# Koukyosyumei/MyZKP

Hardware: AMD Instinct MI355X
Metric: G1 MSM pairs/sec + NTT elems/sec at 2^20 and 2^24; bit-exact vs CPU (higher is better)
Workload: dtype u32x9 (29-bit limbs, 254-bit Montgomery); 1 GPU; KZG commit = BN254 G1 Pippenger MSM of 2^20 (scalar, point) pairs per GPU against a device-resident SRS (commit_kzg, kzg.rs:57-59); 17-bit signed windows (library default at this size), 15 window tables built once at upload; N GPUs = one MSM of N*2^20 pairs (BASELINE configs[2]/[3]); pairs_per_gpu=1048576, seed=332211571536, window_bits=17

## Files before the change

myzkp_amd/csrc/mzk_common.h:

```cpp
#pragma once
#include <hip/hip_runtime.h>
#include <stdint.h>
#include <stddef.h>
#include <stdio.h>
#include <string.h>
#include <functional>
#include <string>
#include <vector>
#include "../../include/mzk.h"
#include "mzk_field.h"
#include "mzk_msm_plan.h"
#include "mzk_ws.h"

namespace mzk {

#ifdef MZK_TUNING
#include <stdlib.h>
static inline int tune_int(const char* name, int dflt) { const char* v = getenv(name); return v ? atoi(v) : dflt; } static inline const char* tune_str(const char* name) { return getenv(name); }
#else
static inline constexpr int tune_int(const char*, int dflt) { return dflt; }
static inline constexpr const char* tune_str(const char*) { return nullptr; }
#endif

void set_error(const char* fmt, ...);
void clear_error();
size_t table_budget_bytes();
int hip_fail(hipError_t e, const char* what, const char* file, int line);
#define MZK_HIP(x)                                                        \
  do {                                                                    \
    hipError_t _e = (x);                                                  \
    if (_e != hipSuccess) return mzk::hip_fail(_e, #x, __FILE__, __LINE__); \
  } while (0)
#define MZK_TRY(x)        \
  do {                    \
    int _rc = (x);        \
    if (_rc != MZK_OK) return _rc; \
  } while (0)

enum AttrFlag { ATTR_FINE_SCATTER4 = 0, ATTR_FINE_SCATTER8, ATTR_DIGITS_LDS, ATTR_SMALL_MSM, ATTR_NTT_LARGE_FR, ATTR_NTT_LARGE_M128, ATTR_NTT_LARGE_M128_2WG, ATTR_MANY_SORT1, ATTR_TAIL_ROW, ATTR_COARSE_STAGED4, ATTR_COARSE_STAGED8, ATTR_COUNT };
struct Context {
  bool ready = false;
  int index = 0;
  int device = -1;
  int num_cu = 256;
  hipStream_t stream = nullptr;
  WsTable ws;
  hipEvent_t ws_event = nullptr;
  hipEvent_t fork_event = nullptr, join_event = nullptr;
  hipStream_t ws_last = nullptr;
  bool ws_used = false;
  bool attr_done[ATTR_COUNT] = {};
  hipStream_t xstream[MZK_MAX_CTX] = {};
  hipEvent_t xdone[MZK_MAX_CTX] = {};
  hipEvent_t xready = nullptr;
  void* bounce = nullptr;
};
constexpr size_t SMALL_D2H_MAX = 4096;
int d2h_sync(void* host, const void* dev, size_t bytes, hipStream_t s);
int ctx_peer_enabled(int a, int b);
struct EntryGuard {
  bool ok;
  bool nested;
  EntryGuard();
  ~EntryGuard();
};
#define MZK_ENTER()                        \
  mzk::EntryGuard _mzk_entry;              \
  if (!_mzk_entry.ok) return MZK_E_BUSY;   \
  MZK_TRY(mzk::ensure_init())
Context& ctx();
int ctx_count();
int ctx_select(int index);
int ensure_init();
struct CtxScope {
  int prev_ctx, prev_dev; bool ok;
  explicit CtxScope(int index);
  ~CtxScope();
};

struct WsGuard {
  hipStream_t s;
  explicit WsGuard(hipStream_t s_);
  ~WsGuard();
};

void prof_begin(hipStream_t s, int phase);
void prof_end(hipStream_t s, int phase);
struct ProfScope {
  hipStream_t s; int ph;
  ProfScope(hipStream_t s_, int ph_) : s(s_), ph(ph_) { prof_begin(s, ph); }
  ~ProfScope() { prof_end(s, ph); }
};
// ... 175 lines not shown
```

myzkp_amd/csrc/mzk_msm.hip:

```cpp
#include <stdlib.h>
#include <type_traits>
#include "mzk_common.h"
#include "mzk_elem.h"
#include "mzk_ec.h"
#include "mzk_coop.h"
#include "mzk_row.h"
#include "mzk_glv.h"
#include "mzk_affine_wave.h"

namespace mzk {

static const MsmKnobs& msm_knobs() {
  static const MsmKnobs k = [] {
    const MsmKnobs d;
    return MsmKnobs{tune_int("MZK_GLV_C", d.glv_c), tune_int("MZK_SMALL_SCAN", d.small_scan), tune_int("MZK_SCAN_MAX_LOG", d.scan_max_log),
                    tune_int("MZK_ACC_SEG", d.acc_seg), tune_int("MZK_COARSE_LOG_20", d.coarse_log_20),
                    tune_int("MZK_COARSE_LOG_17", d.coarse_log_17), tune_int("MZK_PER_FINE", d.per_fine), tune_int("MZK_SORT_SCAN_FREE", d.sort_scan_free),
                    tune_int("MZK_COMBINE_WIDE_MIN_LOG", d.combine_wide_min_log), tune_int("MZK_COMBINE_FORM", d.combine_form),
                    tune_int("MZK_COMBINE_LANE_TPB", d.combine_lane_tpb)};
  }();
  return k;
}

int msm_generic_window_bits(size_t n) { return choose_shape_glv(n ? n : 1, msm_knobs().glv_c).c; }

__device__ __forceinline__ Xyzz xyzz_gload(const u32* __restrict__ g, size_t idx) {
  u32 w[32];
#pragma unroll
  for (int q = 0; q < 4; q++) load_words8(g + idx * 32 + 8 * q, w + 8 * q);
  return xyzz_load(w);
}
__device__ __forceinline__ void xyzz_gstore(u32* __restrict__ g, size_t idx, const Xyzz& p) {
  u32 w[32];
  xyzz_store(p, w);
#pragma unroll
  for (int q = 0; q < 4; q++) store_words8(g + idx * 32 + 8 * q, w + 8 * q);
}

static_assert(SLOT_WORDS == 4 * FqParams::L, "a slot is the four raw coordinates");
__device__ __forceinline__ void xyzz_gstore_raw(u32* __restrict__ g, size_t idx, const Xyzz& p) {
  u32 w[SLOT_WORDS];
  const bool inf = xyzz_is_inf(p);
#pragma unroll
  for (int i = 0; i < FqParams::L; i++) {
    w[i] = inf ? 0u : p.X.l[i]; w[9 + i] = inf ? 0u : p.Y.l[i]; w[18 + i] = inf ? 0u : p.ZZ.l[i]; w[27 + i] = inf ? 0u : p.ZZZ.l[i];
  }
  uint4* p4 = reinterpret_cast<uint4*>(g + idx * SLOT_WORDS);
#pragma unroll
  for (int q = 0; q < SLOT_WORDS / 4; q++) p4[q] = make_uint4(w[4 * q], w[4 * q + 1], w[4 * q + 2], w[4 * q + 3]);
}
__device__ __forceinline__ Xyzz xyzz_gload_raw(const u32* __restrict__ g, size_t idx) {
  u32 w[SLOT_WORDS];
  const uint4* p4 = reinterpret_cast<const uint4*>(g + idx * SLOT_WORDS);
#pragma unroll
  for (int q = 0; q < SLOT_WORDS / 4; q++) { const uint4 v = p4[q]; w[4 * q] = v.x; w[4 * q + 1] = v.y; w[4 * q + 2] = v.z; w[4 * q + 3] = v.w; }
  Xyzz p;
#pragma unroll
  for (int i = 0; i < FqParams::L; i++) { p.X.l[i] = w[i]; p.Y.l[i] = w[9 + i]; p.ZZ.l[i] = w[18 + i]; p.ZZZ.l[i] = w[27 + i]; }
  return p;
}
__device__ __forceinline__ Xyzz xyzz_gload_raw_quad(const u32* __restrict__ g, size_t idx, int lane) {
  Fq mine;
  const u32* src = g + idx * SLOT_WORDS + 9 * lane;
#pragma unroll
  for (int i = 0; i < FqParams::L; i++) mine.l[i] = src[i];
  Xyzz p;
  p.X = quad_bcast<0>(mine);
  p.Y = quad_bcast<1>(mine);
  p.ZZ = quad_bcast<2>(mine);
  p.ZZZ = quad_bcast<3>(mine);
  return p;
}
// ... 370 lines not shown
  for (int k = 0; k < COARSE_PER_WG / SORT2_THREADS; k++) {
    const size_t i = lo + tid + (size_t)k * SORT2_THREADS;
    if (i < hi) load_scalar_canonical(scalars, i, w[k]);
  }
#pragma unroll 1
  for (int k = 0; k < COARSE_PER_WG / SORT2_THREADS; k++) {
    const size_t i = lo + tid + (size_t)k * SORT2_THREADS;
    if (tid < COARSE_BINS) hist[tid] = 0;
    __syncthreads();
    if (i < hi) walk_digits_merged<C>(w[k], table_stride, i, [&](int, u32 key, u32) { counter_inc_agg(hist, key >> key_shift); });
    __syncthreads();
    if (tid < 64) {
      u32 c[PER_LANE], sum = 0;
#pragma unroll
      for (int q = 0; q < PER_LANE; q++) { c[q] = hist[PER_LANE * tid + q]; sum += c[q]; }
      u32 incl = sum;
#pragma unroll
      for (int d = 1; d < 64; d <<= 1) {
        const u32 up = (u32)__shfl_up((int)incl, d, 64);
        if (tid >= d) incl += up;
      }
      u32 run = incl - sum;
#pragma unroll
      for (int q = 0; q < PER_LANE; q++) { loff[PER_LANE * tid + q] = run; run += c[q]; }
      if (tid == 63) loff[COARSE_BINS] = incl;
    }
    __syncthreads();
    if (tid < COARSE_BINS) {
      const u32 cnt = hist[tid];
      if (bin_tot) {
        gpos[tid] = cursor[tid] + (cnt ? atomicAdd(&bin_cur[tid], cnt) : 0u);
      } else {
        gpos[tid] = cursor[tid];
        cursor[tid] += cnt;
      }
      hist[tid] = loff[tid];
    }
    __syncthreads();
    if (i < hi) walk_digits_merged<C>(w[k], table_stride, i, [&](int, u32 key, u32 payload) {
      const u32 bin = key >> key_shift;
      const u32 pos = counter_inc_agg(hist, bin);
      stage[pos] = REC::make(payload, key & fine_mask, fb);
      stage_bin[pos] = (BinTag)bin;
    });
    __syncthreads();
    const u32 total = loff[COARSE_BINS];
    for (u32 p = tid; p < total; p += SORT2_THREADS) {
      const u32 b = stage_bin[p];
      tmp[gpos[b] + (p - loff[b])] = stage[p];
    }
    __syncthreads();
  }
}
struct FineSlice { int bin, s, Sb; u32 lo, hi, start; bool active; };
__device__ __forceinline__ FineSlice fine_plan(const u32* __restrict__ binbase, int nwg, int bins, int S, u32 cap, u32* sc, u32* res) {
  const int tid = threadIdx.x;
  u32 start = 0, len = 0, Sb = 0;
  if (tid < bins) {
    start = binbase[(size_t)tid * nwg];
    len = binbase[(size_t)(tid + 1) * nwg] - start;
    Sb = (len + cap - 1) / cap;
    if (Sb < (u32)S) Sb = (u32)S;
  }
  if (tid == 0) res[0] = 0xffffffffu;
  const int lane = tid & 63, wave = tid >> 6;
  u32 v = Sb;
#pragma unroll
  for (int off = 1; off < 64; off <<= 1) { const u32 t = __shfl_up(v, off, 64); if (lane >= off) v += t; }
  if (lane == 63) sc[wave] = v;
  __syncthreads();
  if (wave == 0) {
    u32 t = (lane < SORT2_THREADS / 64) ? sc[lane] : 0u;
#pragma unroll
    for (int off = 1; off < SORT2_THREADS / 64; off <<= 1) { const u32 u = __shfl_up(t, off, 64); if (lane >= off) t += u; }
    if (lane < SORT2_THREADS / 64) sc[lane] = t;
  }
  __syncthreads();
  const u32 w = blockIdx.x, incl = v + (wave ? sc[wave - 1] : 0u), excl = incl - Sb;
  if (tid < bins && excl <= w && w < incl) { res[0] = (u32)tid; res[1] = w - excl; res[2] = Sb; res[3] = start; res[4] = len; res[5] = excl; }
  __syncthreads();
  FineSlice r;
  r.active = res[0] != 0xffffffffu;
  r.bin = (int)res[0]; r.s = (int)res[1]; r.Sb = (int)res[2];
  const u64 L = res[4];
  r.start = res[3];
  r.lo = res[3] + (u32)(L * (u64)r.s / (u64)r.Sb);
  r.hi = res[3] + (u32)(L * (u64)(r.s + 1) / (u64)r.Sb);
  return r;
}
constexpr int FINE_UNROLL = 8;
template <class REC>
__global__ __launch_bounds__(SORT2_THREADS) void k_fine_count(const typename REC::T* __restrict__ tmp, const u32* __restrict__ binbase, int nwg, int F,
                                                               int S, int fb, u32* __restrict__ finehist, int bins, u32 cap, u32* __restrict__ bucket_tot) {
  __shared__ u32 hist[FINE_MAX];
  __shared__ u32 sc[SORT2_THREADS];
  const FineSlice p = fine_plan(binbase, nwg, bins, S, cap, sc, hist);
  __syncthreads();
  if (!p.active) {
    for (int f = threadIdx.x; f < F; f += SORT2_THREADS) finehist[(size_t)blockIdx.x * F + f] = 0;
    return;
  }
  for (int f = threadIdx.x; f < F; f += SORT2_THREADS) hist[f] = 0;
  __syncthreads();
  const u32 lo = p.lo, hi = p.hi;
  for (u32 base = lo + threadIdx.x; base < hi; base += FINE_UNROLL * SORT2_THREADS) {
    u32 f[FINE_UNROLL];
#pragma unroll
    for (int k = 0; k < FINE_UNROLL; k++) {
      const u32 e = base + k * SORT2_THREADS;
      f[k] = (e < hi) ? REC::fine(tmp[e], (u32)F - 1u, fb) : 0xffffffffu;
    }
#pragma unroll
    for (int k = 0; k < FINE_UNROLL; k++) if (f[k] != 0xffffffffu) counter_inc_agg(hist, f[k]);
  }
  __syncthreads();
  const size_t hbase = (size_t)F * (blockIdx.x - (u32)p.s);
  for (int f = threadIdx.x; f < F; f += SORT2_THREADS) {
    const u32 v = hist[f];
    finehist[hbase + (size_t)f * p.Sb + p.s] = v;
    if (bucket_tot && v) atomicAdd(&bucket_tot[(size_t)p.bin * F + f], v);
  }
}
template <class REC>
__global__ __launch_bounds__(SORT2_THREADS) void k_fine_scatter_direct(const typename REC::T* __restrict__ tmp, const u32* __restrict__ binbase, int nwg, int F,
                                                                 int S, int fb, const u32* __restrict__ finebase, u32* __restrict__ offsets,
                                                                 u32* __restrict__ entries, size_t nbuckets, int bins, u32 cap) {
  __shared__ u32 cursor[FINE_MAX];
  __shared__ u32 sc[SORT2_THREADS];
  const FineSlice p = fine_plan(binbase, nwg, bins, S, cap, sc, cursor);
  __syncthreads();
  if (blockIdx.x == 0 && threadIdx.x == 0) offsets[nbuckets] = finebase[(size_t)F * gridDim.x];
  if (!p.active) return;
  const size_t hbase = (size_t)F * (blockIdx.x - (u32)p.s);
  for (int f = threadIdx.x; f < F; f += SORT2_THREADS) {
    const u32 base = finebase[hbase + (size_t)f * p.Sb + p.s];
    cursor[f] = base;
    if (p.s == 0) offsets[(size_t)p.bin * F + f] = base;
  }
  __syncthreads();
  const u32 lo = p.lo, hi = p.hi;
  for (u32 base = lo + threadIdx.x; base < hi; base += FINE_UNROLL * SORT2_THREADS) {
    typename REC::T r[FINE_UNROLL];
#pragma unroll
    for (int k = 0; k < FINE_UNROLL; k++) {
      const u32 e = base + k * SORT2_THREADS;
      if (e < hi) r[k] = tmp[e];
    }
#pragma unroll
    for (int k = 0; k < FINE_UNROLL; k++)
      if (base + k * SORT2_THREADS < hi) entries[counter_inc_agg(cursor, REC::fine(r[k], (u32)F - 1u, fb))] = REC::payload(r[k], fb);
  }
}

#ifndef MZK_STAGE_CAP
#define MZK_STAGE_CAP 8192
#endif
constexpr int STAGE_CAP = MZK_STAGE_CAP;
constexpr int STAGE_PER_LANE = STAGE_CAP / SORT2_THREADS;
template <class REC>
__global__ __launch_bounds__(SORT2_THREADS) void k_fine_scatter(const typename REC::T* __restrict__ tmp, const u32* __restrict__ binbase, int nwg, int F,
                                                                 int S, int fb, const u32* __restrict__ finebase, u32* __restrict__ offsets,
                                                                 u32* __restrict__ entries, size_t nbuckets, int bins, u32 cap, const u32* __restrict__ bucket_tot,
                                                                 u32* __restrict__ bucket_cur) {
  extern __shared__ u32 lds_fs[];
  u32* gbase = lds_fs;
  u32* cnt = gbase + F;
  u32* lpre = cnt + F;
  u32* scan = lpre + F;
  u32* spay = scan + SORT2_THREADS;
  unsigned short* skey = reinterpret_cast<unsigned short*>(spay + STAGE_CAP);
  const int tid = threadIdx.x;
  const FineSlice p = fine_plan(binbase, nwg, bins, S, cap, scan, gbase);
  __syncthreads();
  if (blockIdx.x == 0 && tid == 0) offsets[nbuckets] = bucket_tot ? binbase[(size_t)bins * nwg] : finebase[(size_t)F * gridDim.x];
  if (!p.active) return;
  const size_t hbase = (size_t)F * (blockIdx.x - (u32)p.s);
  if (bucket_tot) {
    const int per2 = (F + SORT2_THREADS - 1) / SORT2_THREADS;
    u32 local = 0;
    for (int q = 0; q < per2; q++) { const int f = tid * per2 + q; if (f < F) { const u32 v = bucket_tot[(size_t)p.bin * F + f]; cnt[f] = v; local += v; } }
    u32 run = p.start + block_excl_scan<SORT2_THREADS>(local, scan, nullptr);
    for (int q = 0; q < per2; q++) {
      const int f = tid * per2 + q;
      if (f < F) {
        const u32 v = cnt[f];
        const u32 mine = finebase[hbase + (size_t)f * p.Sb + p.s];
        gbase[f] = run + (mine ? atomicAdd(&bucket_cur[(size_t)p.bin * F + f], mine) : 0u);
        if (p.s == 0) offsets[(size_t)p.bin * F + f] = run;
        run += v;
      }
    }
    __syncthreads();
  } else {
    for (int f = tid; f < F; f += SORT2_THREADS) {
      const u32 base = finebase[hbase + (size_t)f * p.Sb + p.s];
      gbase[f] = base;
      if (p.s == 0) offsets[(size_t)p.bin * F + f] = base;
    }
  }
  const u32 lo = p.lo, hi = p.hi;
  const int per = (F + SORT2_THREADS - 1) / SORT2_THREADS;
  for (u32 chunk = lo; chunk < hi; chunk += STAGE_CAP) {
    const u32 cend = (hi - chunk > (u32)STAGE_CAP) ? chunk + STAGE_CAP : hi;
    for (int f = tid; f < F; f += SORT2_THREADS) cnt[f] = 0;
    __syncthreads();
    typename REC::T r[STAGE_PER_LANE];
    u32 rk[STAGE_PER_LANE];
    const u32 fmask = (u32)F - 1u;
#pragma unroll
    for (int k = 0; k < STAGE_PER_LANE; k++) {
      const u32 e = chunk + tid + k * SORT2_THREADS;
      if (e < cend) r[k] = tmp[e];
    }
#pragma unroll
    for (int k = 0; k < STAGE_PER_LANE; k++) rk[k] = (chunk + tid + k * SORT2_THREADS < cend) ? counter_inc_agg(cnt, REC::fine(r[k], fmask, fb)) : 0u;
    __syncthreads();
    u32 local = 0;
    for (int q = 0; q < per; q++) { const int f = tid * per + q; if (f < F) local += cnt[f]; }
    u32 run = block_excl_scan<SORT2_THREADS>(local, scan, nullptr);
    for (int q = 0; q < per; q++) { const int f = tid * per + q; if (f < F) { lpre[f] = run; run += cnt[f]; } }
    __syncthreads();
#pragma unroll
    for (int k = 0; k < STAGE_PER_LANE; k++) {
      if (chunk + tid + k * SORT2_THREADS < cend) {
        const u32 fk = REC::fine(r[k], fmask, fb);
        const u32 pos = lpre[fk] + rk[k];
        spay[pos] = REC::payload(r[k], fb);
        skey[pos] = (unsigned short)fk;
      }
    }
    __syncthreads();
    const u32 m = cend - chunk;
    for (u32 j = tid; j < m; j += SORT2_THREADS) {
      const u32 f = skey[j];
      entries[gbase[f] + (j - lpre[f])] = spay[j];
    }
    __syncthreads();
    for (int f = tid; f < F; f += SORT2_THREADS) gbase[f] += cnt[f];
    __syncthreads();
  }
}

__global__ __launch_bounds__(256) void k_scan_local(const u32* __restrict__ in, u32* __restrict__ out, u32* __restrict__ block_sums, size_t n) {
  __shared__ u32 sh[256];
  const size_t base = (size_t)blockIdx.x * SCAN_BLOCK + (size_t)threadIdx.x * SCAN_ITEMS;
  u32 v[SCAN_ITEMS], sum = 0;
#pragma unroll
  for (int k = 0; k < SCAN_ITEMS; k++) {
    v[k] = (base + k < n) ? in[base + k] : 0u;
    sum += v[k];
  }
  u32 block_total;
  u32 excl = block_excl_scan<256>(sum, sh, &block_total);
  if (threadIdx.x == 255) block_sums[blockIdx.x] = block_total;
#pragma unroll
  for (int k = 0; k < SCAN_ITEMS; k++) {
    if (base + k < n) out[base + k] = excl;
    excl += v[k];
  }
}
__global__ __launch_bounds__(256) void k_scan_finish(u32* __restrict__ offsets, const u32* __restrict__ block_sums, size_t nblocks, size_t n) {
  __shared__ u32 part[4];
  static_assert(SCAN_BLOCK % 256 == 0, "one block index per workgroup");
  const size_t i = (size_t)blockIdx.x * blockDim.x + threadIdx.x;
  const size_t first = (size_t)blockIdx.x * blockDim.x;
  const bool total_wg = first >= n;
  const size_t blk = total_wg ? nblocks : first / SCAN_BLOCK;
  u32 acc = 0;
  for (size_t j = threadIdx.x; j < blk; j += 256) acc += block_sums[j];
#pragma unroll
  for (int d = 32; d >= 1; d >>= 1) acc += (u32)__shfl_xor((int)acc, d, 64);
  if ((threadIdx.x & 63) == 0) part[threadIdx.x >> 6] = acc;
  __syncthreads();
  const u32 pre = part[0] + part[1] + part[2] + part[3];
  if (total_wg) { if (threadIdx.x == 0) offsets[n] = pre; }
  else if (i < n) offsets[i] = offsets[i] + pre;
}

__global__ __launch_bounds__(256) void k_scan_add(u32* __restrict__ offsets, const u32* __restrict__ prefix, size_t nblocks, size_t n) {
  const size_t i = (size_t)blockIdx.x * blockDim.x + threadIdx.x;
  if (i < n) offsets[i] += prefix[i / SCAN_BLOCK];
  else if (i == n) offsets[n] = prefix[nblocks];
}
static int launch_exclusive_scan(const u32* in, u32* out, size_t n, u32* scratch, hipStream_t s) {
  const size_t sb = (n + SCAN_BLOCK - 1) / SCAN_BLOCK;
  hipLaunchKernelGGL(k_scan_local, dim3((unsigned)sb), dim3(256), 0, s, in, out, scratch, n);
  if (sb <= SCAN_DIRECT_BLOCKS) {
    hipLaunchKernelGGL(k_scan_finish, dim3((unsigned)((n + 255) / 256 + 1)), dim3(256), 0, s, out, (const u32*)scratch, sb, n);
  } else {
    MZK_TRY(launch_exclusive_scan((const u32*)scratch, scratch, sb, scratch + sb + 2, s));
    hipLaunchKernelGGL(k_scan_add, dim3((unsigned)(n / 256 + 1)), dim3(256), 0, s, out, (const u32*)scratch, sb, n);
// ... 466 lines not shown
  xyzz_gstore(state, i, p);
}
int msm_build_tables(const void* d_points_mont, size_t n, void* d_tables, int window_bits, hipStream_t s) {
  WsFrame ws("msm_build_tables");
  if (n == 0) return MZK_OK;
  u32* state;
  MZK_TRY(ws.get(WS_XYZZ_TMP, n * 128, (void**)&state));
  const unsigned blocks = (unsigned)((n + 127) / 128);
  MZK_HIP(hipMemcpyAsync(d_tables, d_points_mont, n * 64, hipMemcpyDeviceToDevice, s));
  hipLaunchKernelGGL(k_srs_state_init, dim3(blocks), dim3(128), 0, s, (const u32*)d_points_mont, n, state);
  for (int win = 1; win < msm_table_windows(window_bits); win++) {
    hipLaunchKernelGGL(k_srs_window_step, dim3(blocks), dim3(128), 0, s, state, n, window_bits);
    MZK_TRY(xyzz_batch_to_affine(state, n, (u32*)d_tables + (size_t)win * n * 16, true, s));
  }
  MZK_HIP(hipGetLastError());
  return MZK_OK;
}

struct SortBufs {
  const u32* scalars; u32* binhist; void* tmp; u32* finehist; u32* scan3; u32* offsets; u32* entries;
  u32 *bin_tot, *bin_cur, *bin_start, *bucket_tot, *bucket_cur;
};
template <class REC>
static int sort_records(const MsmPlan& P, const SortBufs& a, hipStream_t s) {
  typedef typename REC::T R;
  const unsigned bins = 1u << P.cl;
#define MZK_STAGED(C, CLOG) hipLaunchKernelGGL((k_coarse_scatter_staged<REC, C, CLOG>), dim3(P.nwg), dim3(SORT2_THREADS), lds, s, a.scalars, P.n, P.L.table_stride, \
                                               P.key_shift, P.fine_mask, P.fb, (const u32*)a.binhist, P.nwg, (R*)a.tmp, (const u32*)a.bin_tot, a.bin_cur, a.bin_start)
#define MZK_DIRECT(C, CLOG) hipLaunchKernelGGL((k_coarse_scatter<REC, C, CLOG>), dim3(P.nwg), dim3(SORT2_THREADS), 0, s, a.scalars, P.n, P.L, P.key_shift, P.fine_mask, \
                                               P.fb, (const u32*)a.binhist, P.nwg, (R*)a.tmp, (const u32*)a.bin_tot, a.bin_cur, a.bin_start)
  if (P.scatter_staged) {
    const size_t lds = stage_lds_bytes(P.coarse_c, P.cl, sizeof(R));
    bool& attr = ctx().attr_done[sizeof(R) == 4 ? ATTR_COARSE_STAGED4 : ATTR_COARSE_STAGED8];
    if (!attr) {
      MZK_HIP(hipFuncSetAttribute((const void*)k_coarse_scatter_staged<REC, 16>, hipFuncAttributeMaxDynamicSharedMemorySize, 160 * 1024));
      MZK_HIP(hipFuncSetAttribute((const void*)k_coarse_scatter_staged<REC, 17>, hipFuncAttributeMaxDynamicSharedMemorySize, 160 * 1024));
      MZK_HIP(hipFuncSetAttribute((const void*)k_coarse_scatter_staged<REC, 20>, hipFuncAttributeMaxDynamicSharedMemorySize, 160 * 1024));
      MZK_HIP(hipFuncSetAttribute((const void*)k_coarse_scatter_staged<REC, 20, 10>, hipFuncAttributeMaxDynamicSharedMemorySize, 160 * 1024));
      MZK_HIP(hipFuncSetAttribute((const void*)k_coarse_scatter_staged<REC, 17, 9>, hipFuncAttributeMaxDynamicSharedMemorySize, 160 * 1024));
      attr = true;
    }
    if (P.coarse_c == 17 && P.cl == 9) MZK_STAGED(17, 9);
    else if (P.coarse_c == 20 && P.cl == 10) MZK_STAGED(20, 10);
    else if (P.coarse_c == 20) MZK_STAGED(20, COARSE_LOG);
    else if (P.coarse_c == 17) MZK_STAGED(17, COARSE_LOG);
    else MZK_STAGED(16, COARSE_LOG);
  }
  else if (P.cl == 10) MZK_DIRECT(0, 10);
  else MZK_DIRECT(0, COARSE_LOG);
#undef MZK_STAGED
#undef MZK_DIRECT
  const u32* bounds = a.bin_tot ? (const u32*)a.bin_start : (const u32*)a.binhist;
  const int bstride = a.bin_tot ? 1 : P.nwg;
  hipLaunchKernelGGL((k_fine_count<REC>), dim3(P.fine_wgs), dim3(SORT2_THREADS), 0, s, (const R*)a.tmp, bounds, bstride, P.F, P.S,
                     P.fb, a.finehist, (int)bins, P.slice_cap, a.bucket_tot);
  if (!P.fine_free) MZK_TRY(launch_exclusive_scan((const u32*)a.finehist, a.finehist, P.own.n_fine, a.scan3, s));
  if (P.F <= STAGE_F_MAX) {
    const size_t lds = ((size_t)3 * P.F + SORT2_THREADS + STAGE_CAP) * 4 + (size_t)STAGE_CAP * 2;
    bool& staged_attr = ctx().attr_done[sizeof(R) == 4 ? ATTR_FINE_SCATTER4 : ATTR_FINE_SCATTER8];
    if (!staged_attr) {
      MZK_HIP(hipFuncSetAttribute((const void*)k_fine_scatter<REC>, hipFuncAttributeMaxDynamicSharedMemorySize, 160 * 1024));
      staged_attr = true;
    }
    hipLaunchKernelGGL((k_fine_scatter<REC>), dim3(P.fine_wgs), dim3(SORT2_THREADS), lds, s, (const R*)a.tmp, bounds, bstride, P.F,
                       P.S, P.fb, (const u32*)a.finehist, a.offsets, a.entries, P.NBtot, (int)bins, P.slice_cap, (const u32*)a.bucket_tot, a.bucket_cur);
  } else {
    hipLaunchKernelGGL((k_fine_scatter_direct<REC>), dim3(P.fine_wgs), dim3(SORT2_THREADS), 0, s, (const R*)a.tmp, bounds, bstride,
                       P.F, P.S, P.fb, (const u32*)a.finehist, a.offsets, a.entries, P.NBtot, (int)bins, P.slice_cap);
  }
  MZK_HIP(hipGetLastError());
  return MZK_OK;
}

static int msm_take_ws(WsFrame& ws, const MsmWsBytes& b, MsmWs* w) {
  const struct { WsSlot slot; size_t bytes; u32** p; } req[] = {
      {WS_MSM_POINTS, b.points, &w->points}, {WS_MSM_COUNTS, b.counts, &w->counts}, {WS_MSM_OFFSETS, b.offsets, &w->offsets},
      {WS_MSM_CURSOR, b.cursor, &w->cursor}, {WS_MSM_ENTRIES, b.entries, &w->entries}, {WS_MSM_SCAN, b.scan, &w->scan},
      {WS_MSM_BUCKETS, b.buckets, &w->buckets}, {WS_MSM_SLOTS, b.slots, &w->slots}, {WS_MSM_WGHIST, b.wghist, &w->wghist}, {WS_MSM_OUT, b.out, &w->out}};
  for (const auto& r : req)
    if (r.bytes) MZK_TRY(ws.get(r.slot, r.bytes, (void**)r.p));
  return MZK_OK;
}
int msm_dev_impl(const void* d_scalars, const void* d_points, size_t n, int point_kind, size_t table_stride, void* d_out,
                 bool out_partial_xyzz, hipStream_t s, const std::function<int()>* points_ready, const MsmChunkCtx* cc) {
  WsFrame ws("msm_dev_impl");
  if (!d_out || ((!d_scalars || !d_points) && n)) { set_error("msm: null pointer"); return MZK_E_ARG; }
  if (cc && (n < SMALL_MAX_N || n > cc->n_alloc)) { set_error("msm: chunk of %zu pairs (chunks hold 4097 .. %zu)", n, cc->n_alloc); return MZK_E_ARG; }
  if (n == 0) {
    if (points_ready) MZK_TRY((*points_ready)());
    MZK_HIP(hipMemsetAsync(d_out, 0, out_partial_xyzz ? 128 : 64, s));
    return MZK_OK;
  }
  const size_t n_shape = cc ? cc->n_total : n, i0 = cc ? cc->i0 : 0;
  const MsmPlan P = msm_plan(n, n_shape, cc ? cc->n_alloc : n, point_kind, table_stride, ctx().num_cu, cc ? cc->K : 0, msm_knobs());
  if (P.err != MZK_OK) { set_error("%s", P.msg); return P.err; }
  MsmWs w = {};
  if (cc) w = *cc->ws;
  else MZK_TRY(msm_take_ws(ws, P.ws, &w));
  const size_t k = cc ? cc->k : 0;
  u32 *pm = w.points, *counts = w.counts, *offsets = w.offsets + k * (P.NBtot + 1), *ranks = w.cursor, *entries = w.entries + k * P.alloc.E, *scan = w.scan,
      *buckets = w.buckets + k * P.NB * 32, *slots = w.slots + k * P.slot_region_words, *wghist = w.wghist, *wsum = w.out;
  const u32* pts = (pm ? pm : (const u32*)d_points) + i0 * 16;
  bool prepared = false;
  auto prepare = [&]() -> int {
    if (prepared) return MZK_OK;
    prepared = true;
    if (points_ready) MZK_TRY((*points_ready)());
    if (!pm) return MZK_OK;
    prof_begin(s, MZK_PH_MSM_PREPARE);
    MZK_TRY(msm_prepare_points((const u32*)d_points + i0 * 16, n, pm + i0 * 16, pm + (n_shape + i0) * 16, s));
    prof_end(s, MZK_PH_MSM_PREPARE);
    return MZK_OK;
  };
  if (P.path == MsmPath::SmallScan) {
    MZK_TRY(prepare());
    prof_begin(s, MZK_PH_MSM_ACCUMULATE);
#define MZK_SCAN_CASE(C) case C: hipLaunchKernelGGL((k_small_accumulate_scan<256, C>), dim3((unsigned)P.NB), dim3(256), 0, s, (const u32*)d_scalars, n, P.L.table_stride, pts, buckets); break;
    switch (P.L.c) { MZK_SCAN_CASE(8) MZK_SCAN_CASE(10) MZK_SCAN_CASE(11) MZK_SCAN_CASE(12) MZK_SCAN_CASE(13) }
// ... 617 lines not shown
```

myzkp_amd/csrc/mzk_msm_plan.h:

```cpp
#pragma once
#include <stddef.h>
#include <stdint.h>
#include <stdio.h>
#include "../../include/mzk.h"

namespace mzk {

enum { MSM_PTS_PLAIN = 0, MSM_PTS_MONT = 1, MSM_PTS_TABLES = 2 };
static inline int msm_table_windows(int c) { return 254 / c + 1; }
static inline int msm_table_rows(int c, int sets) { return 254 / (c * sets) + 1; }

constexpr int SCALAR_BITS = 254;
constexpr int MAX_WINDOWS = 32;
constexpr int GLV_MAG_BITS = 126;
constexpr int SLOT_WORDS = 36;
constexpr int ACC_RESIDENT_WAVES = 3;

struct DigitLayout {
  int c, nwin, merged;
  int sets;
  size_t table_stride;
  int glv;
  size_t phi_offset;
};

struct MsmShape { int c, nwin, lgB; size_t nbuckets; };
static MsmShape choose_shape_glv(size_t n, int force_c = 0) {
  int lg = 0;
  while (((size_t)1 << lg) < 2 * n) lg++;
  int c = lg - 3;
  if (c < 8) c = 8;
  if (c > 16) c = 16;
  if (c == 15) c = 16;
  if (n >= ((size_t)3 << 21)) c = 19;
  if (force_c > 0) c = force_c;
  for (; c > 8; c--) {
    const int nw = GLV_MAG_BITS / c + 1;
    if (GLV_MAG_BITS - c * (nw - 1) >= 5) break;
  }
  MsmShape s;
  s.c = c;
  s.nwin = GLV_MAG_BITS / c + 1;
  s.lgB = c - 1;
  s.nbuckets = (size_t)s.nwin << s.lgB;
  return s;
}

#ifndef MZK_COARSE_LOG
#define MZK_COARSE_LOG 8
#endif
constexpr int COARSE_LOG = MZK_COARSE_LOG;
constexpr int COARSE_PER_WG = 4096;
constexpr int FINE_MAX = 8192;
constexpr int STAGE_F_MAX = 2048;
constexpr size_t SMALL_MAX_N = 4097;
constexpr size_t SMALL_MAX_BUCKETS = 8192;
constexpr int SCAN_ITEMS = 8;
constexpr int SCAN_BLOCK = 256 * SCAN_ITEMS;
constexpr size_t SCAN_DIRECT_BLOCKS = 2048;
static inline size_t scan_scratch_words(size_t n) {
  const size_t sb = (n + SCAN_BLOCK - 1) / SCAN_BLOCK;
  return sb + 2 + (sb > SCAN_DIRECT_BLOCKS ? scan_scratch_words(sb) : 0);
}
constexpr uint32_t HEAVY_SLOTS = 32;
constexpr int HEAVY_GRID = 512;
constexpr int SORT_CTR_BINS = 1024;
constexpr int SORT_CTR_AT = 2 + HEAVY_GRID;
constexpr int HEAVY_HDR = SORT_CTR_AT + 2 * SORT_CTR_BINS;
constexpr size_t heavy_list_words(size_t max_heavy) { return (HEAVY_HDR + 2 * max_heavy + 2 + 3) & ~(size_t)3; }
constexpr size_t heavy_total_words(size_t max_heavy) { return heavy_list_words(max_heavy) + (size_t)HEAVY_GRID * 32 + 8; }

struct MsmKnobs {
  int glv_c = 0;
  int small_scan = 1;
  int scan_max_log = 14;
  int acc_seg = 0;
  int coarse_log_20 = 10;
  int coarse_log_17 = 9;
  int per_fine = 0;
  int sort_scan_free = 3;
  int combine_wide_min_log = 17;
  int combine_form = 0;
  int combine_lane_tpb = 256;
};

enum class MsmPath { SmallScan, SmallSort, TwoLevel, LdsOnePass, Atomic };
struct MsmWsBytes { size_t points, counts, offsets, cursor, entries, buckets, scan, slots, wghist, out; };
struct MsmSizing { size_t E, T, n_coarse, n_fine; };

struct MsmPlan {
  int err = MZK_OK;
  char msg[192] = {};
  size_t n = 0;
  DigitLayout L{};
  int lgB = 0, red_windows = 0, horner_c = 0;
  size_t NB = 0, NBtot = 0;
  bool one_set = false, small_wide = false;
  MsmPath path = MsmPath::SmallSort;
  int cl = 0, F = 0, fb = 0, key_shift = 0, S = 0, nwg = 0;
  uint32_t fine_mask = 0, slice_cap = 0;
  unsigned fine_wgs = 0;
  size_t per_wg = 0;
  bool compact = false, coarse_free = false, fine_free = false, scatter_staged = false;
  int coarse_c = 0;
  uint32_t seg = 0, t_max = 0;
  size_t T = 0, nslots = 0, max_heavy = 0, slot_region_words = 0;
  bool combine_wide = false, combine_ahead = false;
  int combine_tpb = 256;
  MsmSizing own{}, alloc{};
  MsmWsBytes ws{}, ws_used{};
  MsmPlan& fail(const char* fmt, size_t a = 0, size_t b = 0, size_t c = 0) { err = MZK_E_ARG; snprintf(msg, sizeof msg, fmt, a, b, c); return *this; }
};

static inline size_t msm_slot_region_words(size_t T, size_t NB) {
  return ((T + NB + 1) * SLOT_WORDS + heavy_total_words((T + NB) / HEAVY_SLOTS + 1) + 3) & ~(size_t)3;
}
static inline MsmPlan& msm_sized(MsmPlan& P, size_t regions) {
  for (int u = 0; u < 2; u++) {
    const MsmSizing& z = u ? P.own : P.alloc;
    MsmWsBytes& w = u ? P.ws_used : P.ws;
    w.points = P.ws.points, w.out = P.ws.out;
    w.offsets = regions * (P.NBtot + 1) * 4;
    w.entries = regions * z.E * 4;
    w.buckets = regions * P.NB * 128;
    if (P.path == MsmPath::SmallScan || P.path == MsmPath::SmallSort) continue;
    const bool two = P.path == MsmPath::TwoLevel;
    w.counts = 2 * P.NBtot * 4;
    w.cursor = z.E * (two ? 8 : 4);
    w.slots = regions * msm_slot_region_words(z.T, P.NB) * 4;
    w.wghist = two ? (z.n_coarse + 1 + z.n_fine + 1 + ((size_t)1 << P.cl) + 1) * 4 : P.path == MsmPath::LdsOnePass ? (size_t)P.nwg * P.NB * 4 : 0;
    w.scan = two ? (scan_scratch_words(z.n_coarse) + scan_scratch_words(z.n_fine) + 4) * 4 : scan_scratch_words(P.NB) * 4;
  }
  return P;
}

static inline MsmPlan msm_plan(size_t n, size_t n_shape, size_t n_alloc, int point_kind, size_t table_stride, int num_cu, int chunks,
                               const MsmKnobs& kn) {
  MsmPlan P;
  P.n = n;
  if (n > ((size_t)1 << 27)) return P.fail("msm: n > 2^27 not supported");
  const int kind = point_kind & 0xff, table_c = (point_kind >> 8) & 0xff, table_sets = (point_kind >> 16) & 0xff;
  DigitLayout& L = P.L;
  L.merged = kind == MSM_PTS_TABLES;
  L.sets = (L.merged && table_sets) ? table_sets : 1;
  L.table_stride = table_stride;
  L.glv = !L.merged;
  L.phi_offset = kind == MSM_PTS_PLAIN ? n_shape : table_stride;
  const MsmShape sh = choose_shape_glv(n_shape, kn.glv_c);
  L.c = L.merged ? (table_c ? table_c : 16) : sh.c;
  L.nwin = L.merged ? msm_table_windows(L.c) : sh.nwin;
  P.NB = L.merged ? (size_t)L.sets << (L.c - 1) : sh.nbuckets;
  P.lgB = L.c - 1, P.red_windows = L.merged ? L.sets : L.nwin;
  P.one_set = L.merged && L.sets == 1, P.horner_c = P.one_set ? 0 : L.c;
  const size_t windows_per_pair = L.glv ? 2 * L.nwin : L.nwin, regions = chunks ? chunks : 1;
// ... 18 lines not shown
  seg = kn.acc_seg > 0 ? (size_t)kn.acc_seg : seg < 16 ? 16 : seg;
  P.seg = (uint32_t)seg;
  P.T = P.own.T = (E_max + seg - 1) / seg;
  P.t_max = kn.acc_seg > 0 ? 0u : (uint32_t)P.T;
  P.nslots = P.T + P.NB + 1;
  P.max_heavy = (P.T + P.NB) / HEAVY_SLOTS + 1;
  const size_t lanes_fill_chip = (size_t)64 * 4 * (size_t)(num_cu > 0 ? num_cu : 1);
  P.combine_wide = kn.combine_form ? kn.combine_form == 2
                                   : P.NB >= ((size_t)1 << kn.combine_wide_min_log) || (P.one_set && P.NB >= lanes_fill_chip);
  P.combine_ahead = P.combine_wide && P.NB < ((size_t)1 << kn.combine_wide_min_log);
  P.combine_tpb = (kn.combine_lane_tpb == 64 || kn.combine_lane_tpb == 128) ? kn.combine_lane_tpb : 256;
  const size_t T_seg = E_alloc / (kn.acc_seg > 0 ? (size_t)kn.acc_seg : 16) + 1;
  P.alloc.T = !chunks ? P.T : kn.acc_seg > 0 ? T_seg : (resident_lanes + 1 < T_seg ? resident_lanes + 1 : T_seg);
  P.slot_region_words = msm_slot_region_words(P.alloc.T, P.NB);

  const bool plain_merged = L.merged && L.sets == 1;
  P.cl = (plain_merged && L.c == 20 && kn.coarse_log_20 == 10) ? 10 : COARSE_LOG;
  if (plain_merged && L.c == 17 && kn.coarse_log_17 == 9 && COARSE_LOG == 8 && ref_max > ((size_t)1 << (31 - 8)) && ref_max <= ((size_t)1 << (31 - 7)))
    P.cl = 9;
  if (L.glv && P.NBtot > ((size_t)STAGE_F_MAX << COARSE_LOG)) P.cl = 10;
  const size_t cbins = (size_t)1 << P.cl;
  const bool two_level = (P.NBtot & (P.NBtot - 1)) == 0 && P.NBtot >= 4096 && (P.NBtot / cbins) <= (size_t)FINE_MAX &&
                         (n >= 4096 || (L.merged && P.NBtot > ((size_t)1 << 15)));
  if (chunks && !two_level) return P.fail("msm: chunk mode needs the two-level sort (layout %zu bits, %zu buckets)", (size_t)L.c, P.NB);
  P.path = two_level ? MsmPath::TwoLevel : L.merged ? MsmPath::LdsOnePass : MsmPath::Atomic;
  if (P.path == MsmPath::LdsOnePass) {
    const size_t nwg = (n + 4095) / 4096;
    P.nwg = nwg < 1 ? 1 : nwg > (size_t)num_cu ? num_cu : (int)nwg;
    P.per_wg = (n + P.nwg - 1) / P.nwg;
  }
  if (!two_level) return msm_sized(P, regions);
  while (((size_t)1 << P.key_shift) < P.NBtot) P.key_shift++;
  P.key_shift -= P.cl;
  P.F = (int)(P.NBtot / cbins);
  P.fine_mask = (uint32_t)P.F - 1u;
  while ((1 << P.fb) < P.F) P.fb++;
  P.nwg = (int)((n + COARSE_PER_WG - 1) / COARSE_PER_WG);
  const size_t per_fine = kn.per_fine > 0 ? (size_t)kn.per_fine : (P.F >= 4096 ? 131072 : P.F >= 2048 ? 65536 : (L.glv ? 16384 : 32768));
  const size_t S = (E_max / cbins + per_fine - 1) / per_fine;
  P.S = S < 2 ? 2 : S > 64 ? 64 : (int)S;
  const size_t slice_nom = (E_max + cbins * (size_t)P.S - 1) / (cbins * (size_t)P.S);
  P.slice_cap = (uint32_t)(slice_nom + slice_nom / 2 + 1);
  P.fine_wgs = (unsigned)(cbins * (size_t)P.S + (E_max + P.slice_cap - 1) / P.slice_cap + 1);
  P.own.n_coarse = cbins * P.nwg;
  P.own.n_fine = (size_t)P.F * P.fine_wgs;
  const size_t slice_nom_a = (E_alloc + cbins * (size_t)64 - 1) / (cbins * (size_t)64);
  P.alloc.n_coarse = chunks ? cbins * ((n_alloc + COARSE_PER_WG - 1) / COARSE_PER_WG) : P.own.n_coarse;
  P.alloc.n_fine = chunks ? (size_t)P.F * (cbins * 64 + (E_alloc + slice_nom_a) / (slice_nom_a + slice_nom_a / 2 + 1) + 2) : P.own.n_fine;
  P.compact = ref_max <= ((size_t)1 << (31 - P.fb));
  P.coarse_free = (kn.sort_scan_free & 1) != 0 && cbins <= (size_t)SORT_CTR_BINS;
  P.fine_free = (kn.sort_scan_free & 2) != 0 && P.F <= STAGE_F_MAX;
  P.coarse_c = (plain_merged && (L.c == 16 || L.c == 17 || L.c == 20)) ? L.c : 0;
  P.scatter_staged = P.coarse_c != 0;
  return msm_sized(P, regions);
}

#if defined(__HIPCC__)
#define MZK_HD __host__ __device__ __forceinline__
#else
#define MZK_HD inline
#endif
constexpr uint32_t MANY_SENTINEL = 0xffffffffu;

MZK_HD bool seg_span(uint64_t t, uint32_t seg, uint32_t total, uint32_t* e0, uint32_t* e1) {
  const uint64_t e0w = t * seg;
  if (e0w >= total) return false;
  *e0 = (uint32_t)e0w;
  *e1 = (e0w + seg < total) ? (uint32_t)e0w + seg : total;
  return true;
}

template <int K, class Offset>
MZK_HD size_t seg_bucket_search(Offset offset_at, size_t nbuckets, uint32_t e) {
  size_t lo = 0, hi = nbuckets;
  while (hi - lo > 1) {
    const size_t step = (hi - lo + K - 1) / K;
    uint32_t v[K];
#if defined(__HIPCC__)
#pragma unroll
#endif
    for (int j = 1; j < K; j++) v[j] = offset_at(lo + j * step < hi ? lo + j * step : hi);
    size_t below = 0;
#if defined(__HIPCC__)
#pragma unroll
#endif
    for (int j = 1; j < K; j++) below += v[j] <= e ? 1 : 0;
    lo += below * step;
    if (lo + step < hi) hi = lo + step;
  }
  return lo;
}
template <class Offset>
MZK_HD size_t seg_first_bucket(Offset offset_at, size_t nbuckets, uint32_t e) {
  return nbuckets <= ((size_t)1 << 20) ? seg_bucket_search<16>(offset_at, nbuckets, e) : seg_bucket_search<32>(offset_at, nbuckets, e);
}

template <bool SENT, class Entry, class Offset, class IssueRow, class TakeRow, class Flush, class Add>
MZK_HD void seg_walk(uint32_t e0, uint32_t e1, size_t b, size_t nbuckets, Entry entry_at, Offset offset_at, IssueRow issue_row, TakeRow take_row,
                     Flush flush, Add add) {
  const auto row_ref = [](uint32_t ent) { return (SENT && ent == MANY_SENTINEL) ? 0u : ent; };
  const auto end_after_next = [&](size_t bb) { return offset_at(bb + 2 <= nbuckets ? bb + 2 : nbuckets); };
  uint32_t ent = entry_at(e0);
  uint32_t ent1 = entry_at(e1 - e0 > 1 ? e0 + 1 : e0);
  issue_row(row_ref(ent));
  uint32_t bend = offset_at(b + 1), bend1 = end_after_next(b);
  for (uint32_t e = e0; e < e1; e++) {
    take_row(ent);
    const uint32_t ent2 = entry_at(e1 - e > 2 ? e + 2 : e1 - 1);
    issue_row(row_ref(ent1));
    if (e >= bend) {
      flush(b);
      b++, bend = bend1;
      while (e >= bend) b++, bend = offset_at(b + 1);
      bend1 = end_after_next(b);
// ... 79 lines not shown
```

Measured before the change: 786.3 million pairs/s.

## Fuse fine-level bucket sort into one per-bin register-resident kernel

```diff
diff --git a/myzkp_amd/csrc/mzk_common.h b/myzkp_amd/csrc/mzk_common.h
--- a/myzkp_amd/csrc/mzk_common.h
+++ b/myzkp_amd/csrc/mzk_common.h
@@ -37,7 +37,7 @@
     if (_rc != MZK_OK) return _rc; \
   } while (0)
 
-enum AttrFlag { ATTR_FINE_SCATTER4 = 0, ATTR_FINE_SCATTER8, ATTR_DIGITS_LDS, ATTR_SMALL_MSM, ATTR_NTT_LARGE_FR, ATTR_NTT_LARGE_M128, ATTR_NTT_LARGE_M128_2WG, ATTR_MANY_SORT1, ATTR_TAIL_ROW, ATTR_COARSE_STAGED4, ATTR_COARSE_STAGED8, ATTR_COUNT };
+enum AttrFlag { ATTR_FINE_SCATTER4 = 0, ATTR_FINE_SCATTER8, ATTR_DIGITS_LDS, ATTR_SMALL_MSM, ATTR_NTT_LARGE_FR, ATTR_NTT_LARGE_M128, ATTR_NTT_LARGE_M128_2WG, ATTR_MANY_SORT1, ATTR_TAIL_ROW, ATTR_COARSE_STAGED4, ATTR_COARSE_STAGED8, ATTR_FINE_SORT, ATTR_COUNT };
 struct Context {
   bool ready = false;
   int index = 0;
diff --git a/myzkp_amd/csrc/mzk_msm.hip b/myzkp_amd/csrc/mzk_msm.hip
--- a/myzkp_amd/csrc/mzk_msm.hip
+++ b/myzkp_amd/csrc/mzk_msm.hip
@@ -17,7 +17,7 @@
                     tune_int("MZK_ACC_SEG", d.acc_seg), tune_int("MZK_COARSE_LOG_20", d.coarse_log_20),
                     tune_int("MZK_COARSE_LOG_17", d.coarse_log_17), tune_int("MZK_PER_FINE", d.per_fine), tune_int("MZK_SORT_SCAN_FREE", d.sort_scan_free),
                     tune_int("MZK_COMBINE_WIDE_MIN_LOG", d.combine_wide_min_log), tune_int("MZK_COMBINE_FORM", d.combine_form),
-                    tune_int("MZK_COMBINE_LANE_TPB", d.combine_lane_tpb)};
+                    tune_int("MZK_COMBINE_LANE_TPB", d.combine_lane_tpb), tune_int("MZK_FINE_FUSED", d.fine_fused)};
   }();
   return k;
 }
@@ -494,7 +494,6 @@
     __syncthreads();
   }
 }
-struct FineSlice { int bin, s, Sb; u32 lo, hi, start; bool active; };
 __device__ __forceinline__ FineSlice fine_plan(const u32* __restrict__ binbase, int nwg, int bins, int S, u32 cap, u32* sc, u32* res) {
   const int tid = threadIdx.x;
   u32 start = 0, len = 0, Sb = 0;
@@ -528,6 +527,25 @@
   r.start = res[3];
   r.lo = res[3] + (u32)(L * (u64)r.s / (u64)r.Sb);
   r.hi = res[3] + (u32)(L * (u64)(r.s + 1) / (u64)r.Sb);
+  return r;
+}
+__device__ __forceinline__ FineSlice fine_fused_slice(const u32* __restrict__ bound, int bins, u32 cap, u32 j, u32* sc, u32* res) {
+  const int tid = threadIdx.x;
+  u32 start = 0, len = 0;
+  if (tid < bins) {
+    start = bound[tid];
+    len = bound[tid + 1] - start;
+  }
+  if (tid == 0) res[0] = 0u;
+  const u32 excl = block_excl_scan<SORT2_THREADS>(fine_bin_slices(len, cap), sc, nullptr);
+  FineSlice mine;
+  if (tid < bins && fine_slice_of_bin(j, tid, start, len, excl, cap, &mine)) {
+    res[0] = 1u; res[1] = (u32)mine.bin; res[2] = (u32)mine.s; res[3] = (u32)mine.Sb; res[4] = mine.lo; res[5] = mine.hi; res[6] = mine.start;
+  }
+  __syncthreads();
+  FineSlice r;
+  r.active = res[0] != 0u;
+  r.bin = (int)res[1]; r.s = (int)res[2]; r.Sb = (int)res[3]; r.lo = res[4]; r.hi = res[5]; r.start = res[6];
   return r;
 }
 constexpr int FINE_UNROLL = 8;
@@ -603,7 +621,7 @@
 __global__ __launch_bounds__(SORT2_THREADS) void k_fine_scatter(const typename REC::T* __restrict__ tmp, const u32* __restrict__ binbase, int nwg, int F,
                                                                  int S, int fb, const u32* __restrict__ finebase, u32* __restrict__ offsets,
                                                                  u32* __restrict__ entries, size_t nbuckets, int bins, u32 cap, const u32* __restrict__ bucket_tot,
-                                                                 u32* __restrict__ bucket_cur) {
+                                                                 u32* __restrict__ bucket_cur, int fused) {
   extern __shared__ u32 lds_fs[];
   u32* gbase = lds_fs;
   u32* cnt = gbase + F;
@@ -612,9 +630,9 @@
   u32* spay = scan + SORT2_THREADS;
   unsigned short* skey = reinterpret_cast<unsigned short*>(spay + STAGE_CAP);
   const int tid = threadIdx.x;
-  const FineSlice p = fine_plan(binbase, nwg, bins, S, cap, scan, gbase);
-  __syncthreads();
-  if (blockIdx.x == 0 && tid == 0) offsets[nbuckets] = bucket_tot ? binbase[(size_t)bins * nwg] : finebase[(size_t)F * gridDim.x];
+  const FineSlice p = fused ? fine_fused_slice(binbase, bins, cap, blockIdx.x, scan, gbase) : fine_plan(binbase, nwg, bins, S, cap, scan, gbase);
+  __syncthreads();
+  if (!fused && blockIdx.x == 0 && tid == 0) offsets[nbuckets] = bucket_tot ? binbase[(size_t)bins * nwg] : finebase[(size_t)F * gridDim.x];
   if (!p.active) return;
   const size_t hbase = (size_t)F * (blockIdx.x - (u32)p.s);
   if (bucket_tot) {
@@ -679,6 +697,106 @@
     }
     __syncthreads();
     for (int f = tid; f < F; f += SORT2_THREADS) gbase[f] += cnt[f];
+    __syncthreads();
+  }
+}
+
+static_assert(FINE_LANES == SORT2_THREADS && FINE_SORT_F_MAX <= STAGE_F_MAX, "k_fine_sort shares the fine kernels' workgroup and bucket range");
+constexpr size_t fine_sort_lds_bytes(int F) { return ((size_t)F + SORT2_THREADS / 64 + 1 + 7 + ((size_t)1 << FINE_WIN_LOG)) * 4; }
+__global__ __launch_bounds__(SORT2_THREADS, 8) void k_fine_sort(const u32* __restrict__ tmp, const u32* __restrict__ bound, int F, int fb, int bins, u32 cap,
+                                                                 u32* __restrict__ offsets, u32* __restrict__ entries, size_t nbuckets,
+                                                                 u32* __restrict__ finehist, u32* __restrict__ bucket_tot) {
+  extern __shared__ u32 lds_fine[];
+  u32* cnt = lds_fine;
+  u32* sc = cnt + F;
+  u32* res = sc + SORT2_THREADS / 64 + 1;
+  u32* win = res + 7;
+  constexpr u32 WIN = 1u << FINE_WIN_LOG, NOWHERE = 0xffffu, NO_RECORD = 0xffffffffu;
+  constexpr int NPOS = (FINE_REGS + 1) / 2;
+  const u32 tid = threadIdx.x, fmask = (u32)F - 1u;
+  u32 bin;
+  if (fine_wg_is_extra(blockIdx.x, gridDim.x - (u32)bins, &bin)) {
+    const FineSlice p = fine_fused_slice(bound, bins, cap, bin, sc, res);
+    if (!p.active) return;
+    for (u32 f = tid; f < (u32)F; f += SORT2_THREADS) cnt[f] = 0;
+    __syncthreads();
+    for (u32 base = p.lo + tid; base < p.hi; base += FINE_UNROLL * SORT2_THREADS) {
+      u32 f[FINE_UNROLL];
+#pragma unroll
+      for (int k = 0; k < FINE_UNROLL; k++) {
+        const u32 e = base + k * SORT2_THREADS;
+        f[k] = (e < p.hi) ? Rec4::fine(tmp[e], fmask, fb) : 0xffffffffu;
+      }
+#pragma unroll
+      for (int k = 0; k < FINE_UNROLL; k++) if (f[k] != 0xffffffffu) counter_inc_agg(cnt, f[k]);
+    }
+    __syncthreads();
+    const size_t hbase = (size_t)F * (blockIdx.x - (u32)p.s);
+    for (u32 f = tid; f < (u32)F; f += SORT2_THREADS) {
+      const u32 v = cnt[f];
+      finehist[hbase + (size_t)f * p.Sb + p.s] = v;
+      if (v) atomicAdd(&bucket_tot[(size_t)p.bin * F + f], v);
+    }
+    return;
+  }
+  const u32 start = bound[bin], len = bound[bin + 1] - start;
+  if (bin == 0 && tid == 0) offsets[nbuckets] = bound[bins];
+  if (len > FINE_BIN_CAP) return;
+  u32 r[FINE_REGS], pos[NPOS];
+  const u32* mine = tmp + start + tid;
+#pragma unroll
+  for (int k = 0; k < FINE_REGS; k++) {
+    r[k] = NO_RECORD;
+    if (fine_reg_record(k, tid) < len) r[k] = mine[k * FINE_LANES];
+  }
+  if (tid < (u32)F) cnt[tid] = 0;
+  __syncthreads();
+  const auto rank_of = [&](int k) { return r[k] != NO_RECORD ? counter_inc_agg(cnt, Rec4::fine(r[k], fmask, fb)) : NOWHERE; };
+#pragma unroll
+  for (int h = 0; h < NPOS; h++) {
+    const u32 even = rank_of(2 * h), odd = (2 * h + 1 < FINE_REGS) ? rank_of(2 * h + 1) : NOWHERE;
+    pos[h] = even | (odd << 16);
+    asm volatile("" : "+v"(pos[h]));
+    __builtin_amdgcn_sched_barrier(0);
+  }
+  __syncthreads();
+  {
+    const u32 v = tid < (u32)F ? cnt[tid] : 0u;
+    const u32 run = block_excl_scan<SORT2_THREADS>(v, sc, nullptr);
+    if (tid < (u32)F) {
+      cnt[tid] = run;
+      offsets[(size_t)bin * F + tid] = start + run;
+    }
+  }
+  __syncthreads();
+  const auto place_of = [&](int k, u32 rank) {
+    asm volatile("" : "+v"(r[k]));
+    const u32 first = cnt[Rec4::fine(r[k], fmask, fb)];
+    return rank == NOWHERE ? NOWHERE : first + rank;
+  };
+#pragma unroll
+  for (int h = 0; h < NPOS; h++) {
+    const u32 even = place_of(2 * h, pos[h] & 0xffffu), odd = (2 * h + 1 < FINE_REGS) ? place_of(2 * h + 1, pos[h] >> 16) : NOWHERE;
+    pos[h] = even | (odd << 16);
+    asm volatile("" : "+v"(pos[h]));
+    __builtin_amdgcn_sched_barrier(0);
+  }
+#pragma unroll
+  for (int k = 0; k < FINE_REGS; k++) r[k] = Rec4::payload(r[k], fb);
+  for (u32 w0 = 0; w0 < len; w0 += WIN) {
+    const u32 q = w0 >> FINE_WIN_LOG;
+#pragma unroll
+    for (int h = 0; h < NPOS; h++) {
+      u32 both = pos[h];
+      asm volatile("" : "+v"(both));
+      const u32 even = both & 0xffffu, odd = both >> 16;
+      if ((even >> FINE_WIN_LOG) == q) win[even & (WIN - 1u)] = r[2 * h];
+      if (2 * h + 1 < FINE_REGS && (odd >> FINE_WIN_LOG) == q) win[odd & (WIN - 1u)] = r[2 * h + 1];
+    }
+    __syncthreads();
+    const u32 m = (len - w0 < WIN) ? len - w0 : WIN;
+#pragma unroll 2
+    for (u32 j = tid; j < m; j += SORT2_THREADS) entries[start + w0 + j] = win[j];
     __syncthreads();
   }
 }
@@ -1251,18 +1369,34 @@
 #undef MZK_DIRECT
   const u32* bounds = a.bin_tot ? (const u32*)a.bin_start : (const u32*)a.binhist;
   const int bstride = a.bin_tot ? 1 : P.nwg;
+  const size_t scatter_lds = ((size_t)3 * P.F + SORT2_THREADS + STAGE_CAP) * 4 + (size_t)STAGE_CAP * 2;
+  bool& staged_attr = ctx().attr_done[sizeof(R) == 4 ? ATTR_FINE_SCATTER4 : ATTR_FINE_SCATTER8];
+  if (P.F <= STAGE_F_MAX && !staged_attr) {
+    MZK_HIP(hipFuncSetAttribute((const void*)k_fine_scatter<REC>, hipFuncAttributeMaxDynamicSharedMemorySize, 160 * 1024));
+    staged_attr = true;
+  }
+  if constexpr (sizeof(R) == 4) {
+    if (P.fine_fused) {
+      bool& attr = ctx().attr_done[ATTR_FINE_SORT];
+      if (!attr) {
+        MZK_HIP(hipFuncSetAttribute((const void*)k_fine_sort, hipFuncAttributeMaxDynamicSharedMemorySize, 160 * 1024));
+        attr = true;
+      }
+      hipLaunchKernelGGL(k_fine_sort, dim3(P.fine_wgs), dim3(SORT2_THREADS), fine_sort_lds_bytes(P.F), s, (const u32*)a.tmp, (const u32*)a.bin_start, P.F, P.fb,
+                         (int)bins, P.slice_cap, a.offsets, a.entries, P.NBtot, a.finehist, a.bucket_tot);
+      if (P.fine_wgs > bins)
+        hipLaunchKernelGGL((k_fine_scatter<REC>), dim3(P.fine_wgs - bins), dim3(SORT2_THREADS), scatter_lds, s, (const R*)a.tmp, (const u32*)a.bin_start, 1, P.F,
+                           P.S, P.fb, (const u32*)a.finehist, a.offsets, a.entries, P.NBtot, (int)bins, P.slice_cap, (const u32*)a.bucket_tot, a.bucket_cur, 1);
+      MZK_HIP(hipGetLastError());
+      return MZK_OK;
+    }
+  }
   hipLaunchKernelGGL((k_fine_count<REC>), dim3(P.fine_wgs), dim3(SORT2_THREADS), 0, s, (const R*)a.tmp, bounds, bstride, P.F, P.S,
                      P.fb, a.finehist, (int)bins, P.slice_cap, a.bucket_tot);
   if (!P.fine_free) MZK_TRY(launch_exclusive_scan((const u32*)a.finehist, a.finehist, P.own.n_fine, a.scan3, s));
   if (P.F <= STAGE_F_MAX) {
-    const size_t lds = ((size_t)3 * P.F + SORT2_THREADS + STAGE_CAP) * 4 + (size_t)STAGE_CAP * 2;
-    bool& staged_attr = ctx().attr_done[sizeof(R) == 4 ? ATTR_FINE_SCATTER4 : ATTR_FINE_SCATTER8];
-    if (!staged_attr) {
-      MZK_HIP(hipFuncSetAttribute((const void*)k_fine_scatter<REC>, hipFuncAttributeMaxDynamicSharedMemorySize, 160 * 1024));
-      staged_attr = true;
-    }
-    hipLaunchKernelGGL((k_fine_scatter<REC>), dim3(P.fine_wgs), dim3(SORT2_THREADS), lds, s, (const R*)a.tmp, bounds, bstride, P.F,
-                       P.S, P.fb, (const u32*)a.finehist, a.offsets, a.entries, P.NBtot, (int)bins, P.slice_cap, (const u32*)a.bucket_tot, a.bucket_cur);
+    hipLaunchKernelGGL((k_fine_scatter<REC>), dim3(P.fine_wgs), dim3(SORT2_THREADS), scatter_lds, s, (const R*)a.tmp, bounds, bstride, P.F,
+                       P.S, P.fb, (const u32*)a.finehist, a.offsets, a.entries, P.NBtot, (int)bins, P.slice_cap, (const u32*)a.bucket_tot, a.bucket_cur, 0);
   } else {
     hipLaunchKernelGGL((k_fine_scatter_direct<REC>), dim3(P.fine_wgs), dim3(SORT2_THREADS), 0, s, (const R*)a.tmp, bounds, bstride,
                        P.F, P.S, P.fb, (const u32*)a.finehist, a.offsets, a.entries, P.NBtot, (int)bins, P.slice_cap);
diff --git a/myzkp_amd/csrc/mzk_msm_plan.h b/myzkp_amd/csrc/mzk_msm_plan.h
--- a/myzkp_amd/csrc/mzk_msm_plan.h
+++ b/myzkp_amd/csrc/mzk_msm_plan.h
@@ -69,6 +69,69 @@
 constexpr int HEAVY_HDR = SORT_CTR_AT + 2 * SORT_CTR_BINS;
 constexpr size_t heavy_list_words(size_t max_heavy) { return (HEAVY_HDR + 2 * max_heavy + 2 + 3) & ~(size_t)3; }
 constexpr size_t heavy_total_words(size_t max_heavy) { return heavy_list_words(max_heavy) + (size_t)HEAVY_GRID * 32 + 8; }
+constexpr int FINE_LANES = 1024;
+constexpr int FINE_REGS = 33;
+constexpr uint32_t FINE_BIN_CAP = (uint32_t)FINE_REGS * FINE_LANES;
+constexpr int FINE_SORT_F_MAX = 1024;
+constexpr int FINE_WIN_LOG = 14;
+static_assert(FINE_BIN_CAP + (1u << FINE_WIN_LOG) <= 0xffffu, "a record's position in its bin packs into 16 bits, 0xffff falls into no round");
+
+#if defined(__HIPCC__)
+#define MZK_HD __host__ __device__ __forceinline__
+#else
+#define MZK_HD inline
+#endif
+
+struct FineSlice { int bin, s, Sb; uint32_t lo, hi, start; bool active; };
+MZK_HD uint32_t fine_reg_record(int k, uint32_t lane) { return (uint32_t)k * FINE_LANES + lane; }
+MZK_HD bool fine_wg_is_extra(uint32_t w, uint32_t extra, uint32_t* idx) { *idx = w < extra ? w : w - extra; return w < extra; }
+MZK_HD uint32_t fine_bin_slices(uint32_t len, uint32_t cap) { return len > FINE_BIN_CAP ? (uint32_t)(((uint64_t)len + cap - 1) / cap) : 0u; }
+MZK_HD void fine_slice_bounds(uint32_t start, uint32_t len, uint32_t s, uint32_t Sb, uint32_t* lo, uint32_t* hi) {
+  *lo = start + (uint32_t)((uint64_t)len * s / Sb);
+  *hi = start + (uint32_t)((uint64_t)len * (s + 1) / Sb);
+}
+MZK_HD bool fine_slice_of_bin(uint32_t j, int bin, uint32_t start, uint32_t len, uint32_t excl, uint32_t cap, FineSlice* out) {
+  const uint32_t Sb = fine_bin_slices(len, cap);
+  if (j < excl || j - excl >= Sb) return false;
+  out->bin = bin, out->s = (int)(j - excl), out->Sb = (int)Sb, out->start = start, out->active = true;
+  fine_slice_bounds(start, len, j - excl, Sb, &out->lo, &out->hi);
+  return true;
+}
+static inline size_t fine_max_slices(size_t E, size_t bins, uint32_t cap) {
+  const size_t open = (size_t)FINE_BIN_CAP + 1, a = (open + cap - 1) / cap, first = a * cap - FINE_BIN_CAP;
+  size_t best = 0;
+  for (size_t m = 1; m <= bins && m * open <= E; m++) {
+    const size_t rest = E - m * open, cheap = rest / first < m ? rest / first : m;
+    const size_t v = m * a + cheap + (rest - cheap * first) / cap;
+    if (v > best) best = v;
+  }
+  return best;
+}
+constexpr uint64_t FR_TOP64 = 0x30644e72e131a029ull;
+static inline size_t fine_uniform_max_bin(const DigitLayout& L, size_t n, size_t F) {
+  const int nsets = L.merged ? L.sets : L.nwin;
+  double best = 0;
+  for (int set = 0; set < nsets; set++) {
+    double sum = 0;
+    for (int w = 0; w < L.nwin; w++) {
+      if ((L.merged ? w % L.sets : w) != set) continue;
+      double range = (double)((uint64_t)1 << (L.c - 1));
+      if (w == L.nwin - 1) {
+        const int low = L.c * w, top = (L.glv ? GLV_MAG_BITS : 256) - low;
+        const double r = L.glv ? (double)((uint64_t)1 << (top > 0 ? top : 0)) : (double)(FR_TOP64 >> (64 - top)) + 1;
+        if (r < range) range = r;
+      }
+      sum += (double)(L.glv ? 2 * n : n) * (range > (double)F ? (double)F / range : 1.0);
+    }
+    if (sum > best) best = sum;
+  }
+  return (size_t)best + 1;
+}
+static inline bool fine_bins_fit(size_t fullest) {
+  if (fullest >= FINE_BIN_CAP) return false;
+  const size_t margin = FINE_BIN_CAP - fullest;
+  return margin * margin >= 64 * fullest;
+}
 
 struct MsmKnobs {
   int glv_c = 0;
@@ -82,6 +145,7 @@
   int combine_wide_min_log = 17;
   int combine_form = 0;
   int combine_lane_tpb = 256;
+  int fine_fused = -1;
 };
 
 enum class MsmPath { SmallScan, SmallSort, TwoLevel, LdsOnePass, Atomic };
@@ -100,6 +164,7 @@
   int cl = 0, F = 0, fb = 0, key_shift = 0, S = 0, nwg = 0;
   uint32_t fine_mask = 0, slice_cap = 0;
   unsigned fine_wgs = 0;
+  bool fine_fused = false;
   size_t per_wg = 0;
   bool compact = false, coarse_free = false, fine_free = false, scatter_staged = false;
   int coarse_c = 0;
@@ -224,14 +289,15 @@
   P.fine_free = (kn.sort_scan_free & 2) != 0 && P.F <= STAGE_F_MAX;
   P.coarse_c = (plain_merged && (L.c == 16 || L.c == 17 || L.c == 20)) ? L.c : 0;
   P.scatter_staged = P.coarse_c != 0;
+  const bool fused_can = !chunks && P.compact && ref_max < ((size_t)1 << (31 - P.fb)) && P.coarse_free && P.fine_free && P.F <= FINE_SORT_F_MAX;
+  P.fine_fused = fused_can && kn.fine_fused != 0 && (kn.fine_fused > 0 || fine_bins_fit(fine_uniform_max_bin(L, n, (size_t)P.F)));
+  if (P.fine_fused) {
+    P.fine_wgs = (unsigned)(cbins + fine_max_slices(E_max, cbins, P.slice_cap));
+    P.own.n_fine = P.alloc.n_fine = (size_t)P.F * P.fine_wgs;
+  }
   return msm_sized(P, regions);
 }
 
-#if defined(__HIPCC__)
-#define MZK_HD __host__ __device__ __forceinline__
-#else
-#define MZK_HD inline
-#endif
 constexpr uint32_t MANY_SENTINEL = 0xffffffffu;
 
 MZK_HD bool seg_span(uint64_t t, uint32_t seg, uint32_t total, uint32_t* e0, uint32_t* e1) {
```

Result: faster. 800.7 million pairs/s (median of 6 runs) (+1.8%).
